# wvu-navLab/corenav-GP

Hardware: AMD Instinct MI355X
Metric: GP-fits/s (higher is better)
Workload: dtype f64; 1 GPU; BASELINE configs[1]: batch of independent fixed-theta GP fits, N=2048 d=6 M=599 kernel=SE-ARD f64; streams=0, pipeline_depth=1, N=2048, d=6, M=599, inputs=resident in HBM, ranks=1

## Files before the change

corenav_gp_amd/csrc/cgp_kernels_fused.hpp:

```cpp
#pragma once
#include "cgp_kernels.hpp"

namespace cgp {

#ifndef CGP_SKIP_DEAD_WAVE
#define CGP_SKIP_DEAD_WAVE 1
#endif
constexpr bool kSkipDeadWave = CGP_SKIP_DEAD_WAVE != 0;

template <typename T>
__device__ __forceinline__ void stage_first_chunk(const T *gR, size_t ldR, const T *gC, size_t ldC, T *smem, int tid) {
  constexpr int CH = KT * LDST;
  if constexpr (sizeof(T) == 8) {
    typedef __attribute__((address_space(3))) void lds_void;
    typedef const __attribute__((address_space(1))) void gbl_void;
    const int lane = tid & 63;
    const int wave = __builtin_amdgcn_readfirstlane(tid >> 6);
#pragma unroll
    for (int i = 0; i < KT / 4; ++i) {
      const int col = wave * (KT / 4) + i;
      __builtin_amdgcn_global_load_lds((gbl_void *)(gR + (size_t)col * ldR + lane * 2), (lds_void *)(smem + col * LDST), 16, 0, 0);
      __builtin_amdgcn_global_load_lds((gbl_void *)(gC + (size_t)col * ldC + lane * 2), (lds_void *)(smem + CH + col * LDST), 16, 0, 0);
    }
  } else {
// ... 529 lines not shown
  for (int ks = 0; ks < KT / 4; ++ks) asm volatile("" : "+v"(f.r[S][ks]));
  if constexpr (ISSUE) {
    cpanel_stage<T>(gC, ldC, c + D, smem + ((S + D) % R) * CH, lane, wave);
    rfrag_load<T, (S + D) % R>(f, gRl, ldR, c + D, lq);
  }
  const T *cur = smem + S * CH + lq * LDST + l15;
  T fa[2][NCB];
#pragma unroll
  for (int cb = 0; cb < NCB; ++cb) fa[0][cb] = cur[cb * DB];
#pragma unroll
  for (int ks = 0; ks < KT / 4; ++ks) {
    if (ks + 1 < KT / 4) {
#pragma unroll
      for (int cb = 0; cb < NCB; ++cb) fa[(ks + 1) & 1][cb] = cur[(ks + 1) * 4 * LDST + cb * DB];
    }
    const typename RowFrag<T, R>::vec2 fb = f.r[S][ks];
    if constexpr (ACC) {
      const T zv = zs[ks * 4 + lq];
      ms[0] = __builtin_fma(fb[0], zv, ms[0]);
      ms[1] = __builtin_fma(fb[1], zv, ms[1]);
      ms[2] = __builtin_fma(fb[0], fb[0], ms[2]);
      ms[3] = __builtin_fma(fb[1], fb[1], ms[3]);
    }
#pragma unroll
    for (int cb = 0; cb < NCB; ++cb) {
      acc[cb][0] = P::mfma(fa[ks & 1][cb], fb[0], acc[cb][0]);
      acc[cb][1] = P::mfma(fa[ks & 1][cb], fb[1], acc[cb][1]);
    }
  }
}

template <typename T, int R = 4>
__device__ __forceinline__ void mfma_rowpanel_loop_rdirect(typename Prec<T>::acc_t (&acc)[NCB][2], RowFrag<T, R> &f, const T *gR,
                                                           size_t ldR, const T *gC, size_t ldC, int nchunk, T *smem, int tid,
                                                           const T *zs, T (&ms)[4]) {
  if (nchunk <= 0) return;
  constexpr int D = deep_dist<R>();
  constexpr int L = cpanel_loads<T>() + KT / 4;
  static_assert((D - 1) * L <= 63 && D < R && 8 % R == 0, "ring / distance / vmcnt");
  const int lane = tid & 63;
  const int wave = __builtin_amdgcn_readfirstlane(tid >> 6);
  const T *gRl = gR + wave * 32 + 2 * (lane & 15);
  int c = 0;
  for (; c + 8 < nchunk; c += R) {
    static_for<0, R>([&](auto jc) {
      constexpr int J = decltype(jc)::value;
      rdirect_step<T, R, J, true, (D - 1) * L>(acc, f, gRl, ldR, gC, ldC, c + J, smem, lane, wave);
    });
  }
  static_for<0, 8>([&](auto jc) {
    constexpr int J = decltype(jc)::value;
    constexpr int behind = (D - 1) < (7 - J) ? (D - 1) : (7 - J);
    rdirect_step<T, R, J % R, (J + D < 8), behind * L, true>(acc, f, gRl, ldR, gC, ldC, c + J, smem, lane, wave, zs + J * KT, ms);
  });
}

constexpr int TRI_PD = 2;
__device__ __forceinline__ constexpr int tri_buf(int i) { return i * KT * LDST; }

template <typename T> constexpr int tri_dma_loads() { return sizeof(T) == 8 ? KT / 4 : KT / 2; }
template <typename T, bool DEEP = sizeof(T) == 8>
__device__ __forceinline__ void stage_chunk_tri(const T *gR, size_t ldR, int chunk, T *buf, int tid) {
  if constexpr (DEEP) {
    typedef __attribute__((address_space(3))) void lds_void;
    typedef const __attribute__((address_space(1))) void gbl_void;
    const int lane = tid & 63;
    const int wave = __builtin_amdgcn_readfirstlane(tid >> 6);
#pragma unroll
    for (int i = 0; i < KT / 4; ++i) {
      const int col = wave * (KT / 4) + i;
      const T *src = gR + (size_t)(chunk * KT + col) * ldR;
      if constexpr (sizeof(T) == 8) {
        __builtin_amdgcn_global_load_lds((gbl_void *)(src + lane * 2), (lds_void *)(buf + col * LDST), 16, 0, 0);
      } else {
        __builtin_amdgcn_global_load_lds((gbl_void *)(src + lane), (lds_void *)(buf + col * LDST), 4, 0, 0);
        __builtin_amdgcn_global_load_lds((gbl_void *)(src + 64 + lane), (lds_void *)(buf + col * LDST + 64), 4, 0, 0);
      }
    }
  } else {
    using vec8 = T __attribute__((ext_vector_type(8)));
    const int sc = tid >> 4, sr = (tid & 15) * 8;
    *reinterpret_cast<vec8 *>(buf + sc * LDST + sr) = *reinterpret_cast<const vec8 *>(gR + sr + (size_t)(chunk * KT + sc) * ldR);
  }
}

template <typename T, int W, bool DEEP>
__device__ __forceinline__ void syrk_tri_wave(typename Prec<T>::acc_t (&acc)[NCB][2], const T *gR, size_t ldR, int nchunk,
                                              T *smem, int tid) {
  using P = Prec<T>;
  constexpr int RB0 = W, RB1 = NCB - 1 - W;
  const int lane = tid & 63;
  const int l15 = lane & 15, lq = lane >> 4;

  auto compute = [&](const T *cur) {
#pragma unroll
    for (int ks = 0; ks < KT / 4; ++ks) {
      const T *ra = cur + (ks * 4 + lq) * LDST + l15;
      T fa[RB1 + 1];
#pragma unroll
      for (int cb = 0; cb <= RB1; ++cb) fa[cb] = ra[cb * DB];
#pragma unroll
      for (int cb = 0; cb <= RB1; ++cb) {
        if (cb <= RB0) acc[cb][0] = P::mfma(fa[cb], fa[RB0], acc[cb][0]);
        acc[cb][1] = P::mfma(fa[cb], fa[RB1], acc[cb][1]);
      }
    }
// ... 96 lines not shown
  const bf8 c01[2] = {__builtin_bit_cast(bf8, a01[RB0]), __builtin_bit_cast(bf8, a01[RB1])};
  static_for<0, RB1 + 1>([&](auto cc) {
    constexpr int CB = decltype(cc)::value;
    const bf8 a = __builtin_bit_cast(bf8, a01[CB]);
    if constexpr (CB <= RB0) acc[CB][0] = __builtin_amdgcn_mfma_f32_16x16x32_bf16(a, c10[0], acc[CB][0], 0, 0, 0);
    acc[CB][1] = __builtin_amdgcn_mfma_f32_16x16x32_bf16(a, c10[1], acc[CB][1], 0, 0, 0);
  });
  static_for<0, RB1 + 1>([&](auto cc) {
    constexpr int CB = decltype(cc)::value;
    const bf8 a = __builtin_bit_cast(bf8, a01[CB]);
    if constexpr (CB <= RB0) acc[CB][0] = __builtin_amdgcn_mfma_f32_16x16x32_bf16(a, c01[0], acc[CB][0], 0, 0, 0);
    acc[CB][1] = __builtin_amdgcn_mfma_f32_16x16x32_bf16(a, c01[1], acc[CB][1], 0, 0, 0);
  });
}
template <int D, int W, int S>
__device__ __forceinline__ void bx6_tri_iter(Prec<float>::acc_t (&acc)[NCB][2], BxTriStage<D> &st, int c, int nchunk, float *smem, const unsigned (&e)[2], bool hi) {
  st.template load<S>(c + D);
  lds_barrier();
  bx6_tri_compute<W, (S & 1) * 6 * BX_PLANE>(acc, e, hi);
  if (c + 1 < nchunk) st.template store<(S + 1) % D>(smem + ((S + 1) & 1) * BXT_FLOATS);
}
template <int D, int W>
__device__ __forceinline__ void bx6_tri_wave(Prec<float>::acc_t (&acc)[NCB][2], BxTriStage<D> &st, int nchunk, float *smem, int tid) {
  const int lane = tid & 63, l15 = lane & 15, lq = lane >> 4;
  const unsigned base = (unsigned)(size_t)smem;
  const unsigned e[2] = {base + 2 * bx_pos(l15, lq & 1), base + 2 * (bx_pos(DB + l15, lq & 1) - DB * BXS)};
  st.template store<0>(smem);
  for (int c0 = 0; c0 < nchunk; c0 += D) {
    bx6_tri_iter<D, W, 0>(acc, st, c0, nchunk, smem, e, lq >> 1);
    bx6_tri_iter<D, W, 1>(acc, st, c0 + 1, nchunk, smem, e, lq >> 1);
    if (D > 2) bx6_tri_iter<D, W, 2 % D>(acc, st, c0 + 2, nchunk, smem, e, lq >> 1);
    if (D > 2) bx6_tri_iter<D, W, 3 % D>(acc, st, c0 + 3, nchunk, smem, e, lq >> 1);
  }
}
template <int D>
__device__ __forceinline__ void bx6_syrk_tri_loop(Prec<float>::acc_t (&acc)[NCB][2], BxTriStage<D> &st, int nchunk, float *smem, int tid) {
  if (nchunk <= 0) return;
  const int wave = __builtin_amdgcn_readfirstlane(tid >> 6);
  switch (wave) {
    case 0: bx6_tri_wave<D, 0>(acc, st, nchunk, smem, tid); break;
    case 1: bx6_tri_wave<D, 1>(acc, st, nchunk, smem, tid); break;
    case 2: bx6_tri_wave<D, 2>(acc, st, nchunk, smem, tid); break;
    default: bx6_tri_wave<D, 3>(acc, st, nchunk, smem, tid); break;
  }
}

__device__ __forceinline__ double exp_gen(double x, const ExpC &e) { return exp_nonpos(x, e); }
__device__ __forceinline__ float exp_gen(float x, const ExpC &) { return __expf(fmaxf(x, -104.f)); }

constexpr int GK = 12;
template <bool DBL> constexpr int bx_z_offset() { return DBL ? 2 * BX_FLOATS : BX_FLOATS + 2 * GK * TS + 3 * TS; }
static_assert(2 * GK * TS + 3 * TS <= BX_FLOATS, "Gram inputs fit the second plane buffer");

template <typename T, bool BROWN, bool FAST, bool TRI = false, int NR = 2, bool DIFF1 = false, int MAT = 0>
__device__ __forceinline__ void gram_apply_tile(const FitArgs &p, typename Prec<T>::acc_t (&acc)[NCB][NR],
                                                const T *__restrict__ xrT, const T *__restrict__ xcT,
                                                const T *__restrict__ xraw, const T *__restrict__ craw,
                                                const T *__restrict__ yc, bool extra, int rowbase, int colbase, T amp,
                                                T amp_b, T diag_add, int lane, int wave, T inv_ell = T(0)) {
  using P = Prec<T>;
  using acc_t = typename P::acc_t;
  const int N = p.N, M = p.M, l15 = lane & 15, lq = lane >> 4;
  ExpC ec;
  ec.load();
  static_assert(NR == 2 || (NR == 1 && !TRI), "row blocks per wave");
  const int rbj[2] = {TRI ? wave : 0, TRI ? NCB - 1 - wave : 0};
  const int rl[2] = {TRI ? rbj[0] * DB + l15 : (NR == 2 ? wave * 32 + 2 * l15 : wave * DB + l15),
                     TRI ? rbj[1] * DB + l15 : wave * 32 + 2 * l15 + 1};
  T fb[NR][GK / 4];
#pragma unroll
  for (int j = 0; j < NR; ++j)
#pragma unroll
    for (int s = 0; s < GK / 4; ++s) fb[j][s] = xrT[(4 * s + lq) * TS + rl[j]];
  static_assert(!DIFF1 || (!BROWN && sizeof(T) == 4), "the difference form is for the fp32 SE kernels");
  static_assert(MAT == 0 || (!BROWN && !DIFF1 && sizeof(T) == 8), "the Matern kernels are fp64 cases of the inner-product form");
  T xrw[2] = {T(0), T(0)};
  if (BROWN || DIFF1) {
    xrw[0] = xraw[rl[0]];
    if (NR == 2) xrw[1] = xraw[rl[1]];
  }
#pragma unroll
  for (int cb = 0; cb < NCB; ++cb) {
    if (TRI && cb > rbj[0] && cb > rbj[1]) continue;
    T fa[GK / 4];
#pragma unroll
    for (int s = 0; s < GK / 4; ++s) fa[s] = xcT[(4 * s + lq) * TS + cb * DB + l15];
#pragma unroll
    for (int j = 0; j < NR; ++j) {
      if (TRI && cb > rbj[j]) continue;
      acc_t e = acc_t{0, 0, 0, 0};
      if constexpr (!DIFF1) {
#pragma unroll
        for (int s = 0; s < GK / 4; ++s) e = P::mfma(fa[s], fb[j][s], e);
      }
      const int grow = rowbase + rl[j];
#pragma unroll
      for (int r = 0; r < 4; ++r) {
        const int cl = cb * DB + P::drow(lane, r);
        const int gcol = colbase + cl;
        T g;
        if constexpr (DIFF1) {
          const T df = (xrw[j] - craw[cl]) * inv_ell;
          g = amp * exp_gen(T(-0.5) * df * df, ec);
        } else if constexpr (MAT != 0) {
          const bool same = !FAST && !extra && grow == gcol;
          double unused;
          g = amp * T(matern_radial<MAT == 2, false>(same ? 0.0 : -2.0 * (double)e[r], unused, [&](double x) { return exp_nonpos(x, ec); }));
        } else if (!BROWN) {
          g = CGP_DBG_ON(p, 128) ? e[r] : exp_gen(e[r], ec);
        } else {
          const T x = xrw[j], xp = craw[cl];
          const bool same = !FAST && !extra && grow == gcol;
          T ee = e[r] > T(0) ? T(0) : e[r];
          if constexpr (sizeof(T) == 4) {
            const T df = (x - xp) * inv_ell;
            ee = T(-0.5) * df * df;
          }
          ee = same ? T(0) : ee;
          const int sx = (x > T(0)) - (x < T(0)), sp = (xp > T(0)) - (xp < T(0));
          const T ax = x < T(0) ? -x : x, ap = xp < T(0) ? -xp : xp;
          const T kb = (sx == sp) ? amp_b * (ax < ap ? ax : ap) : T(0);
          g = amp * exp_gen(ee, ec) * kb;
        }
        if (!FAST) {
          const bool colok = gcol < N;
          if (!extra) {
            const bool dg = grow == gcol;
            g = dg ? g + diag_add : g;
            g = (grow < N && colok) ? g : (dg ? T(1) : T(0));
          } else {
            if (p.xid) g = (grow == gcol) ? T(1) : T(0);
            g = (grow == M) ? yc[cl] : g;
            g = (!colok || grow > M) ? T(0) : g;
          }
        }
        acc[cb][j][r] = -g;
      }
    }
    __builtin_amdgcn_sched_barrier(0);
  }
}

__global__ void k_prep(FitArgs p, int batch, double *prep, int zero_info, int *wready) {
  const int b = blockIdx.x * blockDim.x + threadIdx.x;
  if (b >= batch) return;
  if (zero_info) p.info[b] = 0;
  if (wready) wready[b] = 0;
  const double *th = p.theta + (size_t)b * MAX_THETA;
  double *o = prep + (size_t)b * PREP_N;
  const int kid = p.kernel_id, d = p.d;
  for (int q = 0; q < MAXD; ++q) {
    double s = 0.0;
    if (q < d) s = k_is_ard(kid) ? 1.0 / th[1 + q] : 1.0 / th[1];
    o[q] = s;
  }
  const bool brown = kid == K_RBF_BROWNIAN;
  o[8] = (brown || k_is_matern(kid)) ? 0.0 : log(th[0]);
  o[9] = th[0];
  o[10] = brown ? th[2] : 0.0;
  const int nth = k_ntheta(kid, d);
  o[11] = th[nth - 1] + 1e-8 + (p.jitter ? p.jitter[b] : 0.0);
  for (int q = 12; q < PREP_N; ++q) o[q] = 0.0;
}

template <typename T> struct GramPre {
  T v[MAXD];
  T yv;
};

template <typename T>
__device__ __forceinline__ void gram_prefetch(const FitArgs &p, int b, int k, int rt, int tid, GramPre<T> &g, int row0 = -1) {
  const int d = p.d, N = p.N, M = p.M;
  const bool extra = rt >= p.NT;
  const T *__restrict__ Xb = reinterpret_cast<const T *>(p.X) + (size_t)b * d * N;
  const T *__restrict__ Xsb = reinterpret_cast<const T *>(p.Xs) + (size_t)b * d * M;
  const T *__restrict__ yb = reinterpret_cast<const T *>(p.y) + (size_t)b * N;
  const bool isrow = tid < TS;
  const int r = tid & 127;
  const T *src = Xb;
  int idx, len = N;
  if (isrow) {
    if (!extra) idx = (row0 >= 0 ? row0 : rt * TS) + r;
    else { src = Xsb; idx = (row0 >= 0 ? row0 : (rt - p.NT) * TS) + r; len = M; }
  } else idx = k * TS + r;
  const bool ok = idx < len;
#pragma unroll
  for (int q = 0; q < MAXD; ++q) g.v[q] = (q < d && ok) ? src[(size_t)q * len + idx] : T(0);
  g.yv = (!isrow && ok) ? yb[idx] : T(0);
}

template <typename T, bool TRI = false, int NR = 2, bool MAT = false>
__device__ __forceinline__ void gram_apply(const FitArgs &p, typename Prec<T>::acc_t (&acc)[NCB][NR], T *__restrict__ smem,
                                           int b, int k, int rt, int tid, const GramPre<T> &g, PhaseClock *pc = nullptr,
                                           int slot = 0, int row0 = -1, bool live = true) {
  const double *__restrict__ pr = p.prep + (size_t)b * PREP_N;
  const int kid = p.kernel_id, N = p.N, M = p.M;
  const bool extra = rt >= p.NT;
  const bool brown = kid == K_RBF_BROWNIAN;
  const int lane = tid & 63;
  const int wave = __builtin_amdgcn_readfirstlane(tid >> 6);
  T *xrT = smem;
  T *xcT = smem + GK * TS;
  T *xraw = smem + 2 * GK * TS;
  T *craw = xraw + TS;
  T *yc = craw + TS;
  {
    const bool isrow = tid < TS;
    const int r = tid & 127;
    T *dst = isrow ? xrT : xcT;
    T nrm = 0;
#pragma unroll
    for (int q = 0; q < MAXD; ++q) {
      const T v = g.v[q] * T(pr[q]);
      nrm = __builtin_fma(v, v, nrm);
      dst[q * TS + r] = v;
    }
    dst[MAXD * TS + r] = isrow ? (T(-0.5) * nrm + T(pr[8])) : T(1);
    dst[(MAXD + 1) * TS + r] = isrow ? T(1) : T(-0.5) * nrm;
    dst[(MAXD + 2) * TS + r] = T(0);
    dst[(MAXD + 3) * TS + r] = T(0);
    if (isrow) xraw[r] = g.v[0];
    else {
      craw[r] = g.v[0];
      yc[r] = g.yv;
    }
  }
  __syncthreads();
  if (pc) pc->lap(p, slot);
  const T amp = T(pr[9]), amp_b = T(pr[10]), diag_add = T(pr[11]);
  const int rowbase = row0 >= 0 ? row0 : (extra ? (rt - p.NT) * TS : rt * TS);
  const int colbase = k * TS;
  constexpr int ROWS = NR == 2 ? TS : TS / 2;
  const bool fast = (colbase + TS <= N) && (extra ? (rowbase + ROWS <= M && !p.xid) : (rt != k && rowbase + ROWS <= N));
  if (!live) return;
  if constexpr (sizeof(T) == 4) {
    if (!brown && p.d == 1) {
      if constexpr (TRI) gram_apply_tile<T, false, false, true, NR, true>(p, acc, xrT, xcT, xraw, craw, yc, extra, rowbase, colbase, amp, amp_b, diag_add, lane, wave, T(pr[0]));
      else if (fast) gram_apply_tile<T, false, true, false, NR, true>(p, acc, xrT, xcT, xraw, craw, yc, extra, rowbase, colbase, amp, amp_b, diag_add, lane, wave, T(pr[0]));
      else gram_apply_tile<T, false, false, false, NR, true>(p, acc, xrT, xcT, xraw, craw, yc, extra, rowbase, colbase, amp, amp_b, diag_add, lane, wave, T(pr[0]));
      return;
    }
  }
  static_assert(!MAT || sizeof(T) == 8, "the Matern kernels are fp64 only");
  if constexpr (MAT) {
#define CGP_MATERN_TILE(FAST_, TRI_)                                                                                                  \
  do {                                                                                                                                \
    if (kid == K_MATERN52_ARD)                                                                                                        \
      gram_apply_tile<T, false, FAST_, TRI_, NR, false, 2>(p, acc, xrT, xcT, xraw, craw, yc, extra, rowbase, colbase, amp, amp_b, diag_add, lane, wave); \
    else                                                                                                                              \
      gram_apply_tile<T, false, FAST_, TRI_, NR, false, 1>(p, acc, xrT, xcT, xraw, craw, yc, extra, rowbase, colbase, amp, amp_b, diag_add, lane, wave); \
  } while (0)
    if constexpr (TRI) CGP_MATERN_TILE(false, true);
    else if (fast) CGP_MATERN_TILE(true, false);
    else CGP_MATERN_TILE(false, false);
#undef CGP_MATERN_TILE
    return;
  }
  if constexpr (TRI) {
    if (brown) gram_apply_tile<T, true, false, true>(p, acc, xrT, xcT, xraw, craw, yc, extra, rowbase, colbase, amp, amp_b, diag_add, lane, wave, T(pr[0]));
    else gram_apply_tile<T, false, false, true>(p, acc, xrT, xcT, xraw, craw, yc, extra, rowbase, colbase, amp, amp_b, diag_add, lane, wave);
  } else if (brown) {
    if (fast) gram_apply_tile<T, true, true, false, NR>(p, acc, xrT, xcT, xraw, craw, yc, extra, rowbase, colbase, amp, amp_b, diag_add, lane, wave, T(pr[0]));
    else gram_apply_tile<T, true, false, false, NR>(p, acc, xrT, xcT, xraw, craw, yc, extra, rowbase, colbase, amp, amp_b, diag_add, lane, wave, T(pr[0]));
  } else {
    if (fast) gram_apply_tile<T, false, true, false, NR>(p, acc, xrT, xcT, xraw, craw, yc, extra, rowbase, colbase, amp, amp_b, diag_add, lane, wave);
    else gram_apply_tile<T, false, false, false, NR>(p, acc, xrT, xcT, xraw, craw, yc, extra, rowbase, colbase, amp, amp_b, diag_add, lane, wave);
  }
}

__device__ __forceinline__ constexpr int tri_blk(int i, int j) { return (i * (i + 1) / 2 + j) * DB * DB; }
template <typename T> constexpr int diag_lds_elems() { return 36 * DB * DB + 3 * DB * DB; }

template <typename T>
__device__ __forceinline__ void diag_factor_packed(const FitArgs &p, T *__restrict__ Bk, T *__restrict__ tile, int ld,
                                                   T *__restrict__ Wk, int b, int k, int tid) {
  using P = Prec<T>;
  using acc_t = typename P::acc_t;
  constexpr int NB = TS / DB;
  const int lane = tid & 63;
  const int wave = __builtin_amdgcn_readfirstlane(tid >> 6);
  const int l15 = lane & 15, lq = lane >> 4;
  const int live = p.N - k * TS;
  T *Dv = Bk + 36 * DB * DB;
  T *DvT = Dv + DB * DB;
  int bad = 0;
  for (int jb = 0; jb < NB; ++jb) {
    const int j0 = jb * DB;
    if (wave == 0) {
      T *Djj = Bk + tri_blk(jb, jb);
      T a[DB], w[DB];
      if (j0 < live) {
#pragma unroll
        for (int c = 0; c < DB; ++c) a[c] = Djj[c * DB + l15];
        factor_block16<T>(a, w, bad, k * TS + j0, l15, [&] {
#pragma unroll
          for (int c = 0; c < DB; ++c) a[c] = Djj[c * DB + l15];
        });
      } else {
#pragma unroll
        for (int c = 0; c < DB; ++c) a[c] = w[c] = (c == l15) ? T(1) : T(0);
      }
      if (lane < DB) {
        T *dvt = DvT + (jb & 1) * DB * DB;
#pragma unroll
        for (int i = 0; i < DB; ++i) {
          Dv[l15 * DB + i] = w[i];
          dvt[i * DB + l15] = w[i];
          Wk[wimg_blk(jb, jb) + l15 * DB + i] = -w[i];
        }
#pragma unroll
        for (int c = 0; c < DB; ++c) tile[(size_t)(j0 + c) * ld + j0 + l15] = (l15 >= c) ? a[c] : T(0);
      }
    } else if (jb > 0) {
      const int pj = jb - 1;
      const T *dvt = DvT + (pj & 1) * DB * DB;
      for (int i = jb + wave - 1; i < NB; i += 3) {
        T *blk = Bk + tri_blk(i, pj);
        T fa[4], fb[4];
#pragma unroll
// ... 360 lines not shown
  for (int cb = 0; cb < NCB; ++cb)
#pragma unroll
    for (int r = 0; r < 4; ++r) {
      vec2 v;
      v[0] = acc[cb][0][r];
      v[1] = acc[cb][1][r];
      *reinterpret_cast<vec2 *>(out + (size_t)(cb * DB + P::drow(lane, r)) * ld) = v;
    }
}
template <typename T, bool ADD>
__device__ __forceinline__ void load_tile(typename Prec<T>::acc_t (&acc)[NCB][2], const T *tile, int ld, int tid) {
  using P = Prec<T>;
  using vec2 = T __attribute__((ext_vector_type(2)));
  const int lane = tid & 63, l15 = lane & 15;
  const int wave = __builtin_amdgcn_readfirstlane(tid >> 6);
  const T *src = tile + wave * 32 + 2 * l15;
#pragma unroll
  for (int cb = 0; cb < NCB; ++cb)
#pragma unroll
    for (int r = 0; r < 4; ++r) {
      const vec2 v = *reinterpret_cast<const vec2 *>(src + (size_t)(cb * DB + P::drow(lane, r)) * ld);
      acc[cb][0][r] = ADD ? acc[cb][0][r] + v[0] : v[0];
      acc[cb][1][r] = ADD ? acc[cb][1][r] + v[1] : v[1];
    }
}


template <typename T, bool DEEP, bool MAT = false>
__device__ __forceinline__ void panel_partial(const FitArgs &p, typename Prec<T>::acc_t (&acc)[NCB][2], T *__restrict__ smem, int b,
                                              int k, int tid) {
  constexpr int CH2 = 2 * KT * LDST;
  const int kc = k + 1, rt = k + 2, ld = p.ld, nchunk = k * (TS / KT);
  const T *Lw = reinterpret_cast<const T *>(p.Lw) + (size_t)b * p.lw_stride;
  const T *gR = Lw + (size_t)rt * TS, *gC = Lw + (size_t)kc * TS;
  GramPre<T> gp;
  gram_prefetch<T>(p, b, kc, rt, tid, gp);
  if constexpr (DEEP) {
    constexpr int R = deep_ring<T, true>();
    RowFrag<T, R> rf;
    T *zs = smem + R * KT * LDST;
    if (tid < TS) zs[tid] = T(0);
    T ms[4] = {T(0), T(0), T(0), T(0)};
    rdirect_prologue<T, R>(rf, gR, (size_t)ld, gC, (size_t)ld, nchunk, smem, tid);
    gram_apply<T, false, 2, MAT>(p, acc, smem + (R - 2) * KT * LDST, b, kc, rt, tid, gp);
    mfma_rowpanel_loop_rdirect<T, R>(acc, rf, gR, (size_t)ld, gC, (size_t)ld, nchunk, smem, tid, zs, ms);
  } else {
    if (nchunk > 0) stage_first_chunk<T>(gR, (size_t)ld, gC, (size_t)ld, smem, tid);
    gram_apply<T, false, 2, MAT>(p, acc, smem + CH2, b, kc, rt, tid, gp);
    mfma_rowpanel_loop<T, true>(acc, gR, (size_t)ld, gC, (size_t)ld, nchunk, smem, tid);
  }
  acc_image<T, false, true>(acc, reinterpret_cast<T *>(p.pimg) + ((size_t)b * img_slots(p) + kc % img_slots(p)) * DPART, tid);
}

#ifndef CGP_IMG_EARLY
#define CGP_IMG_EARLY 1
#endif
template <typename T, bool MID> constexpr bool mid_fat() { return MID && sizeof(T) == 4; }
template <typename T, bool DIAGNEXT, bool DEEP, bool MID, bool MAT = false>
__device__ __forceinline__ void panel_tile_body(const FitArgs &p, int k, int b, int rt, int c_first, bool finish_next, bool from_image,
                                                T *smem, int tid) {
  using P = Prec<T>;
  using acc_t = typename P::acc_t;
  acc_t acc[NCB][2];
  T *Lw = reinterpret_cast<T *>(p.Lw) + (size_t)b * p.lw_stride;
  const int ld = p.ld;
  PhaseClock pc;
  pc.start(p, tid);
  const int ps = finish_next ? 336 : 64 + 8 * (k & 31);

  constexpr int CH2 = 2 * KT * LDST;
  const T *gR = Lw + (size_t)rt * TS + (size_t)(c_first * KT) * ld, *gC = Lw + (size_t)k * TS + (size_t)(c_first * KT) * ld;
  if (CGP_DBG_ON(p, 4096)) gR = reinterpret_cast<const T *>(p.Lw) + (size_t)(b & 7) * p.lw_stride + (size_t)p.NT * TS;
  if (CGP_DBG_ON(p, 8192)) gC = reinterpret_cast<const T *>(p.Lw) + (size_t)(b & 7) * p.lw_stride + (size_t)k * TS;
  const int nchunk = k * (TS / KT) - c_first;
  const T *pimg = reinterpret_cast<const T *>(p.pimg) + ((size_t)b * img_slots(p) + k % img_slots(p)) * DPART;
  const bool accm = p.macc != nullptr && rt >= p.NT && k > 0;
  const bool live = !(kSkipDeadWave && !DEEP && sizeof(T) == 4 && rt >= p.NT && !p.xid &&
                      (rt - p.NT) * TS + __builtin_amdgcn_readfirstlane(tid >> 6) * 32 > p.M);
  constexpr int R = DEEP ? deep_ring<T, MID>() : 4;
  constexpr bool BX6 = kF32Bf16x6 && sizeof(T) == 4 && (!DEEP || MID);
  constexpr bool BXDBL = DEEP;
  constexpr int BXD = DEEP ? kBxMidSets : 1;
  constexpr bool PL = kMidPlanes && BX6 && MID;
  constexpr int GRAM_OFF = PL ? 2 * BXP_BUF / 4 : (BX6 ? BX_FLOATS : CH2);
  T *zs = smem + (PL ? BXP_NBUF * BXP_BUF / 4 : (BX6 ? bx_z_offset<BXDBL>() : R * KT * LDST));
  if (tid < TS) zs[tid] = accm ? Lw[(size_t)((k - 1) * TS + tid) * ld + (size_t)p.NT * TS + p.M] : T(0);
  T ms[4] = {T(0), T(0), T(0), T(0)};
  if constexpr (DEEP && !BX6) {
    RowFrag<T, R> rf;
    {
      GramPre<T> gp;
      if (!(MID && from_image)) gram_prefetch<T>(p, b, k, rt, tid, gp);
      rdirect_prologue<T, R>(rf, gR, (size_t)ld, gC, (size_t)ld, nchunk, smem, tid);
      if (MID && from_image) acc_image<T, false, false>(acc, const_cast<T *>(pimg), tid);
      else gram_apply<T, false, 2, MAT>(p, acc, smem + (R - 2) * KT * LDST, b, k, rt, tid, gp, &pc, ps + 6);
    }
    pc.lap(p, ps + 0);
    mfma_rowpanel_loop_rdirect<T, R>(acc, rf, gR, (size_t)ld, gC, (size_t)ld, nchunk, smem, tid, zs, ms);
  } else {
    BxStage<PL ? 1 : BXD> bxs;
    BxPlaneSrc bps;
    {
      GramPre<T> gp;
      if (!(MID && from_image)) gram_prefetch<T>(p, b, k, rt, tid, gp);
      if (nchunk > 0) {
        if constexpr (PL) {
          bps.init(reinterpret_cast<const unsigned short *>(p.Lp) + (size_t)b * p.lp_stride, p.lp_stride / 3, ld, c_first, rt, k, tid);
          const int wv = __builtin_amdgcn_readfirstlane(tid >> 6);
          bps.issue(0, reinterpret_cast<unsigned char *>(smem), 0, wv);
          bps.issue(1, reinterpret_cast<unsigned char *>(smem), BXP_BUF, wv);
        } else if constexpr (BX6) {
          bxs.init(gR, (size_t)ld, gC, (size_t)ld, nchunk, tid);
          bx6_prologue(bxs, nchunk);
        } else stage_first_chunk<T>(gR, (size_t)ld, gC, (size_t)ld, smem, tid);
      }
      if (CGP_DBG_ON(p, 16384)) {
#pragma unroll
        for (int cb = 0; cb < NCB; ++cb)
#pragma unroll
          for (int j = 0; j < 2; ++j)
#pragma unroll
            for (int r = 0; r < 4; ++r) acc[cb][j][r] = gp.v[0];
      } else if (MID && from_image) acc_image<T, false, false>(acc, const_cast<T *>(pimg), tid);
      else gram_apply<T, false, 2, MAT>(p, acc, smem + GRAM_OFF, b, k, rt, tid, gp, &pc, ps + 6, -1, live);
    }
    pc.lap(p, ps + 0);
    if constexpr (PL) bx6p_loop(acc, bps, nchunk, smem, tid, accm ? zs : nullptr, ms, live, gR, (size_t)ld);
    else if constexpr (BX6) bx6_loop<BXD, BXDBL>(acc, bxs, nchunk, smem, tid, accm ? zs : nullptr, ms, live);
    else mfma_rowpanel_loop<T, true>(acc, gR, (size_t)ld, gC, (size_t)ld, nchunk, smem, tid, accm ? zs : nullptr, ms, live);
  }
  pc.lap(p, ps + 1);
  if (accm) {
#pragma unroll
    for (int q = 0; q < 4; ++q) {
      ms[q] += __shfl_xor(ms[q], 16);
      ms[q] += __shfl_xor(ms[q], 32);
    }
    const int lane = tid & 63;
    const int wave = __builtin_amdgcn_readfirstlane(tid >> 6);
    if (lane < 16) {
#pragma unroll
      for (int j = 0; j < 2; ++j) {
        const int m = (rt - p.NT) * TS + wave * 32 + 2 * lane + j;
        if (m < p.M) {
          double *pm = p.macc + (size_t)b * p.M + m, *pv = p.vacc + (size_t)b * p.M + m;
          const double om = k == 1 ? 0.0 : __hip_atomic_load(pm, __ATOMIC_RELAXED, __HIP_MEMORY_SCOPE_AGENT);
          const double ov = k == 1 ? 0.0 : __hip_atomic_load(pv, __ATOMIC_RELAXED, __HIP_MEMORY_SCOPE_AGENT);
          __hip_atomic_store(pm, om + (double)ms[j], __ATOMIC_RELAXED, __HIP_MEMORY_SCOPE_AGENT);
          __hip_atomic_store(pv, ov + (double)ms[2 + j], __ATOMIC_RELAXED, __HIP_MEMORY_SCOPE_AGENT);
        }
      }
    }
  }
  __syncthreads();
  pc.lap(p, ps + 2);
  if (!CGP_DBG_ON(p, 64)) {
    if constexpr (kF32Bf16x6 && kBxTrmm && sizeof(T) == 4) trmm_bx6(p, acc, smem, b, k, tid, &pc, ps + 3, live);
    else trmm_in_registers<T>(p, acc, smem, b, k, tid, &pc, ps + 3, live);
  }
  pc.lap(p, ps + 4);
  if (live && (!CGP_DBG_ON(p, 32768) || acc[0][0][0] == T(12345.678)))
  store_tile<T>(acc, Lw + (size_t)(k * TS) * ld + (size_t)rt * TS, ld, tid);
  if constexpr (PL) {
    if (live) store_tile_planes(acc, reinterpret_cast<unsigned short *>(p.Lp) + (size_t)b * p.lp_stride, p.lp_stride / 3, ld, rt, k, tid);
  }
  pc.lap(p, ps + 5);
  pc.count(p, ps + 7);
  if constexpr (DIAGNEXT) {
    if (finish_next) {
      bool img_ready = false;
      if constexpr (MID && CGP_IMG_EARLY) {
        if (k + 1 >= 3) {
          const T *img = reinterpret_cast<const T *>(p.dpart) + ((size_t)b * img_slots(p) + (k + 1) % img_slots(p)) * DPART;
          acc_image<T, kTriDiag, false>(acc, const_cast<T *>(img), tid);
          img_ready = true;
        }
      }
      diag_next<T, DIAG_FINISH, kTriDiag, DEEP, mid_fat<T, MID>(), MAT>(p, acc, smem, Lw, b, k + 1, tid, &pc, img_ready);
    }
  }
}

#ifndef CGP_KINDA_PRIO
#define CGP_KINDA_PRIO 0
#endif
#ifndef CGP_F32_FULL_OCC
#define CGP_F32_FULL_OCC 4
#endif
constexpr int F32_FULL_OCC = CGP_F32_FULL_OCC;
template <typename T, bool DIAGNEXT = false, bool DEEP = sizeof(T) == 8, bool MID = false, bool MAT = false>
__global__ __launch_bounds__(256, sizeof(T) == 4 ? (DEEP ? ((MID && (CGP_MID_RING > 4 || CGP_F32_BF16X6)) ? 2 : 3) : F32_FULL_OCC) : 2) void k_panel(FitArgs p, int k) {
  using P = Prec<T>;
  using acc_t = typename P::acc_t;
  extern __shared__ __attribute__((aligned(16))) char smem_raw[];
  T *smem = reinterpret_cast<T *>(smem_raw);
  const int tid = threadIdx.x;
// ... 4 lines not shown
  SpanClock sc;
  sc.enter(p, k, tid);
  if constexpr (DIAGNEXT) {
    const int Tg = gridDim.x, B = gridDim.y;
    const int lin = blockIdx.y * Tg + blockIdx.x;
    const int nA = (p.diag_slots & 1) ? B : 0, nB = (p.diag_slots & 2) ? B : 0, nC = (MID && (p.diag_slots & 4)) ? B : 0;
    int ia = -1, io = lin;
    const int stride = p.diag_stride, ablk = nA >> 8, oblk = (Tg * B - nA) >> 8;
    if (nA > 0 && (B & 255) == 0 && stride > 0 && (ablk - 1) * stride < ablk + oblk) {
      const int j = lin >> 8, r = lin & 255;
      const int before = min((j + stride - 1) / stride, ablk);
      if (j % stride == 0 && j / stride < ablk) ia = (j / stride) * 256 + r;
      else io = (j - before) * 256 + r;
    } else if (lin < nA) ia = lin;
    else io = lin - nA;
    if (CGP_DBG_ON(p, 65536) && (ia >= 0 || io < nB)) {
      if (ia < 0) return;
    }
    if (ia >= 0) {
      b = ia;
      rt = k + 1;
      finish_next = !CGP_DBG_ON(p, 65536);
      if constexpr (MID && CGP_KINDA_PRIO > 0) __builtin_amdgcn_s_setprio(CGP_KINDA_PRIO);
      if (MID && (p.diag_slots & 8)) {
        from_image = true;
        c_first = (k - 1) * (TS / KT);
      }
    } else if (io < nB) {
      b = io;
      T *LwB = reinterpret_cast<T *>(p.Lw) + (size_t)b * p.lw_stride;
      diag_next<T, DIAG_PARTIAL, kTriDiag, DEEP, false, MAT>(p, acc, smem, LwB, b, k + 2, tid);
      sc.leave(p, k, tid);
      return;
    } else if (MID && io < nB + nC) {
      panel_partial<T, DEEP, MAT>(p, acc, smem, io - nB, k, tid);
      sc.leave(p, k, tid);
      return;
    } else {
      const int l2 = io - nB - nC, To = Tg - (nA ? 1 : 0) - (nB ? 1 : 0) - (nC ? 1 : 0);
      if ((B & 7) == 0) {
        const int xcd = l2 & 7, slot = l2 >> 3;
        bt = slot % To;
        b = (slot / To) * 8 + xcd;
      } else {
        bt = l2 % To;
        b = l2 / To;
      }
      const int first = k + 1 + (nA ? 1 : 0);
      const int nin = p.NT - first > 0 ? p.NT - first : 0;
      rt = bt < nin ? first + bt : p.NT + (bt - nin);
    }
  } else {
    tile_fit_of_block(bt, b);
    rt = row_tile_of(bt + p.tile_off, k + 1, p.NT, p.rows_from_extra);
  }
  panel_tile_body<T, DIAGNEXT, DEEP, MID, MAT>(p, k, b, rt, c_first, finish_next, from_image, smem, tid);
  sc.leave(p, k, tid);
}

constexpr int HR = TS / 2;
template <typename T, int SLOT>
__device__ __forceinline__ void r16_load(T (&f)[4][KT / 4], const T *gRl, size_t ldR, int chunk, int lq) {
#pragma unroll
  for (int ks = 0; ks < KT / 4; ++ks) {
    const T *src = gRl + (size_t)(chunk * KT + ks * 4 + lq) * ldR;
    if constexpr (sizeof(T) == 8) asm volatile("global_load_dwordx2 %0, %1, off" : "=&v"(f[SLOT][ks]) : "v"(src));
    else asm volatile("global_load_dword %0, %1, off" : "=&v"(f[SLOT][ks]) : "v"(src));
  }
}
template <typename T, int S, bool ISSUE, int WAITN, bool ACC>
__device__ __forceinline__ void r16_step(typename Prec<T>::acc_t (&acc)[NCB][1], T (&f)[4][KT / 4], const T *gRl, size_t ldR, const T *gC,
                                         size_t ldC, int c, T *smem, int lane, int wave, const T *zs, T *ms) {
  using P = Prec<T>;
  constexpr int CH = KT * LDST;
  const int l15 = lane & 15, lq = lane >> 4;
  asm volatile("s_waitcnt vmcnt(%0)\n\ts_barrier" ::"n"(WAITN) : "memory");
#pragma unroll
  for (int ks = 0; ks < KT / 4; ++ks) asm volatile("" : "+v"(f[S][ks]));
  if constexpr (ISSUE) {
    cpanel_stage<T>(gC, ldC, c + 2, smem + ((S + 2) & 3) * CH, lane, wave);
    r16_load<T, (S + 2) & 3>(f, gRl, ldR, c + 2, lq);
  }
  const T *cur = smem + S * CH + lq * LDST + l15;
  T fa[2][NCB];
#pragma unroll
  for (int cb = 0; cb < NCB; ++cb) fa[0][cb] = cur[cb * DB];
#pragma unroll
  for (int ks = 0; ks < KT / 4; ++ks) {
    if (ks + 1 < KT / 4) {
#pragma unroll
      for (int cb = 0; cb < NCB; ++cb) fa[(ks + 1) & 1][cb] = cur[(ks + 1) * 4 * LDST + cb * DB];
    }
    const T fb = f[S][ks];
    if constexpr (ACC) {
      const T zv = zs[ks * 4 + lq];
      ms[0] = __builtin_fma(fb, zv, ms[0]);
      ms[1] = __builtin_fma(fb, fb, ms[1]);
    }
#pragma unroll
    for (int cb = 0; cb < NCB; ++cb) acc[cb][0] = P::mfma(fa[ks & 1][cb], fb, acc[cb][0]);
  }
}

template <typename T, bool MAT = false>
__global__ __launch_bounds__(256, sizeof(T) == 4 ? 4 : 2) void k_rows64(FitArgs p, int k) {
  using P = Prec<T>;
// ... 686 lines not shown
```

Measured before the change: 11250 fits/s.

## Transpose last partial extra tile update to skip dead row blocks

```diff
diff --git a/corenav_gp_amd/csrc/cgp_kernels_fused.hpp b/corenav_gp_amd/csrc/cgp_kernels_fused.hpp
--- a/corenav_gp_amd/csrc/cgp_kernels_fused.hpp
+++ b/corenav_gp_amd/csrc/cgp_kernels_fused.hpp
@@ -605,6 +605,121 @@
     constexpr int J = decltype(jc)::value;
     constexpr int behind = (D - 1) < (7 - J) ? (D - 1) : (7 - J);
     rdirect_step<T, R, J % R, (J + D < 8), behind * L, true>(acc, f, gRl, ldR, gC, ldC, c + J, smem, lane, wave, zs + J * KT, ms);
+  });
+}
+
+#ifndef CGP_LAST_TILE_COLDEAL
+#define CGP_LAST_TILE_COLDEAL 1
+#endif
+constexpr bool kLastTileColDeal = CGP_LAST_TILE_COLDEAL != 0;
+#ifndef CGP_LAST_TILE_ORDER
+#define CGP_LAST_TILE_ORDER 0
+#endif
+__device__ __forceinline__ int coldeal_blocks(const FitArgs &p, int k) {
+  const int nb = 2 * ((p.M + 1 - (p.ET - 1) * TS + 31) / 32);
+  return (kLastTileColDeal && k >= 1 && p.ET > 0 && !p.rows_from_extra && nb <= 6) ? nb : 0;
+}
+
+template <typename T, int NB, int R, int S, bool ISSUE, int WAITN, bool ACC = false>
+__device__ __forceinline__ void coldeal_step(typename Prec<T>::acc_t (&acc)[NB][2], RowFrag<T, R> &f, const T *gCl, size_t ldC,
+                                             const T *gR, size_t ldR, int c, T *smem, int lane, int wave,
+                                             const T *zs = nullptr, T *ms = nullptr) {
+  using P = Prec<T>;
+  constexpr int CH = KT * LDST;
+  constexpr int D = deep_dist<R>();
+  const int l15 = lane & 15, lq = lane >> 4;
+  static_assert(WAITN >= 0 && WAITN <= 63, "vmcnt is a 6-bit counter");
+  asm volatile("s_waitcnt vmcnt(%0)\n\ts_barrier" ::"n"(WAITN) : "memory");
+#pragma unroll
+  for (int ks = 0; ks < KT / 4; ++ks) asm volatile("" : "+v"(f.r[S][ks]));
+  if constexpr (ISSUE) {
+    cpanel_stage<T>(gR, ldR, c + D, smem + ((S + D) % R) * CH, lane, wave);
+    rfrag_load<T, (S + D) % R>(f, gCl, ldC, c + D, lq);
+  }
+  const T *cur = smem + S * CH + lq * LDST + l15;
+  T fa[2][NB];
+#pragma unroll
+  for (int rb = 0; rb < NB; ++rb) fa[0][rb] = cur[rb * DB];
+#pragma unroll
+  for (int ks = 0; ks < KT / 4; ++ks) {
+    if (ks + 1 < KT / 4) {
+#pragma unroll
+      for (int rb = 0; rb < NB; ++rb) fa[(ks + 1) & 1][rb] = cur[(ks + 1) * 4 * LDST + rb * DB];
+    }
+    const typename RowFrag<T, R>::vec2 fb = f.r[S][ks];
+    if constexpr (ACC) {
+      const T zv = zs[ks * 4 + lq];
+      const T v0 = cur[ks * 4 * LDST + wave * DB], v1 = cur[ks * 4 * LDST + (wave + 4) * DB];
+      ms[0] = __builtin_fma(v0, zv, ms[0]);
+      ms[1] = __builtin_fma(v1, zv, ms[1]);
+      ms[2] = __builtin_fma(v0, v0, ms[2]);
+      ms[3] = __builtin_fma(v1, v1, ms[3]);
+    }
+#pragma unroll
+    for (int rb = 0; rb < NB; ++rb) {
+      acc[rb][0] = P::mfma(fa[ks & 1][rb], fb[0], acc[rb][0]);
+      acc[rb][1] = P::mfma(fa[ks & 1][rb], fb[1], acc[rb][1]);
+    }
+  }
+}
+
+template <typename T, int NB, int R = 4>
+__device__ __forceinline__ void mfma_coldeal_loop(typename Prec<T>::acc_t (&acc)[NB][2], RowFrag<T, R> &f, const T *gR, size_t ldR,
+                                                  const T *gC, size_t ldC, int nchunk, T *smem, int tid, const T *zs, T (&ms)[4]) {
+  if (nchunk <= 0) return;
+  constexpr int D = deep_dist<R>();
+  constexpr int L = cpanel_loads<T>() + KT / 4;
+  static_assert((D - 1) * L <= 63 && D < R && 8 % R == 0, "ring / distance / vmcnt");
+  static_assert(NB >= 2 && NB < NCB && NB % 2 == 0, "live row blocks, rounded up to even");
+  const int lane = tid & 63;
+  const int wave = __builtin_amdgcn_readfirstlane(tid >> 6);
+  const T *gCl = gC + wave * 32 + 2 * (lane & 15);
+  int c = 0;
+  for (; c + 8 < nchunk; c += R) {
+    static_for<0, R>([&](auto jc) {
+      constexpr int J = decltype(jc)::value;
+      coldeal_step<T, NB, R, J, true, (D - 1) * L>(acc, f, gCl, ldC, gR, ldR, c + J, smem, lane, wave);
+    });
+  }
+  static_for<0, 8>([&](auto jc) {
+    constexpr int J = decltype(jc)::value;
+    constexpr int behind = (D - 1) < (7 - J) ? (D - 1) : (7 - J);
+    coldeal_step<T, NB, R, J % R, (J + D < 8), behind * L, true>(acc, f, gCl, ldC, gR, ldR, c + J, smem, lane, wave, zs + J * KT, ms);
+  });
+}
+
+template <typename T, int NB>
+__device__ __forceinline__ void coldeal_to_rows(typename Prec<T>::acc_t (&acc)[NCB][2], const typename Prec<T>::acc_t (&cd)[NB][2],
+                                                T *__restrict__ smem, int tid) {
+  using P = Prec<T>;
+  using vec2 = T __attribute__((ext_vector_type(2)));
+  constexpr int LDX = NB * DB + 2;
+  static_assert(64 * LDX <= 4 * KT * LDST, "a pass fits the chunk ring");
+  const int lane = tid & 63, l15 = lane & 15;
+  const int wave = __builtin_amdgcn_readfirstlane(tid >> 6);
+  const bool rows_live = wave * 32 < NB * DB;
+  const T *rowside = smem + wave * 32 + 2 * l15;
+  T *colside = smem + ((wave & 1) * 32 + 2 * l15) * LDX;
+  static_for<0, 2>([&](auto hc) {
+    constexpr int H = decltype(hc)::value;
+    if ((wave >> 1) == H) {
+#pragma unroll
+      for (int rb = 0; rb < NB; ++rb)
+#pragma unroll
+        for (int j = 0; j < 2; ++j)
+#pragma unroll
+          for (int r = 0; r < 4; ++r) colside[j * LDX + rb * DB + P::drow(lane, r)] = cd[rb][j][r];
+    }
+    lds_barrier();
+#pragma unroll
+    for (int cb = 0; cb < 4; ++cb)
+#pragma unroll
+      for (int r = 0; r < 4; ++r) {
+        const vec2 v = rows_live ? *reinterpret_cast<const vec2 *>(rowside + (cb * DB + P::drow(lane, r)) * LDX) : vec2{T(0), T(0)};
+        acc[4 * H + cb][0][r] = v[0];
+        acc[4 * H + cb][1][r] = v[1];
+      }
+    lds_barrier();
   });
 }
 
@@ -807,6 +922,49 @@
 template <bool DBL> constexpr int bx_z_offset() { return DBL ? 2 * BX_FLOATS : BX_FLOATS + 2 * GK * TS + 3 * TS; }
 static_assert(2 * GK * TS + 3 * TS <= BX_FLOATS, "Gram inputs fit the second plane buffer");
 
+template <typename T, bool BROWN, bool FAST, bool DIFF1, int MAT>
+__device__ __forceinline__ T gram_entry(const FitArgs &p, T ev, T xr, int grow, int cl, int gcol, const T *__restrict__ craw,
+                                        const T *__restrict__ yc, bool extra, T amp, T amp_b, T diag_add, T inv_ell, const ExpC &ec) {
+  const int N = p.N, M = p.M;
+  T g;
+  if constexpr (DIFF1) {
+    const T df = (xr - craw[cl]) * inv_ell;
+    g = amp * exp_gen(T(-0.5) * df * df, ec);
+  } else if constexpr (MAT != 0) {
+    const bool same = !FAST && !extra && grow == gcol;
+    double unused;
+    g = amp * T(matern_radial<MAT == 2, false>(same ? 0.0 : -2.0 * (double)ev, unused, [&](double x) { return exp_nonpos(x, ec); }));
+  } else if (!BROWN) {
+    g = CGP_DBG_ON(p, 128) ? ev : exp_gen(ev, ec);
+  } else {
+    const T x = xr, xp = craw[cl];
+    const bool same = !FAST && !extra && grow == gcol;
+    T ee = ev > T(0) ? T(0) : ev;
+    if constexpr (sizeof(T) == 4) {
+      const T df = (x - xp) * inv_ell;
+      ee = T(-0.5) * df * df;
+    }
+    ee = same ? T(0) : ee;
+    const int sx = (x > T(0)) - (x < T(0)), sp = (xp > T(0)) - (xp < T(0));
+    const T ax = x < T(0) ? -x : x, ap = xp < T(0) ? -xp : xp;
+    const T kb = (sx == sp) ? amp_b * (ax < ap ? ax : ap) : T(0);
+    g = amp * exp_gen(ee, ec) * kb;
+  }
+  if (!FAST) {
+    const bool colok = gcol < N;
+    if (!extra) {
+      const bool dg = grow == gcol;
+      g = dg ? g + diag_add : g;
+      g = (grow < N && colok) ? g : (dg ? T(1) : T(0));
+    } else {
+      if (p.xid) g = (grow == gcol) ? T(1) : T(0);
+      g = (grow == M) ? yc[cl] : g;
+      g = (!colok || grow > M) ? T(0) : g;
+    }
+  }
+  return g;
+}
+
 template <typename T, bool BROWN, bool FAST, bool TRI = false, int NR = 2, bool DIFF1 = false, int MAT = 0>
 __device__ __forceinline__ void gram_apply_tile(const FitArgs &p, typename Prec<T>::acc_t (&acc)[NCB][NR],
                                                 const T *__restrict__ xrT, const T *__restrict__ xcT,
@@ -815,7 +973,7 @@
                                                 T amp_b, T diag_add, int lane, int wave, T inv_ell = T(0)) {
   using P = Prec<T>;
   using acc_t = typename P::acc_t;
-  const int N = p.N, M = p.M, l15 = lane & 15, lq = lane >> 4;
+  const int l15 = lane & 15, lq = lane >> 4;
   ExpC ec;
   ec.load();
   static_assert(NR == 2 || (NR == 1 && !TRI), "row blocks per wave");
@@ -852,44 +1010,50 @@
 #pragma unroll
       for (int r = 0; r < 4; ++r) {
         const int cl = cb * DB + P::drow(lane, r);
-        const int gcol = colbase + cl;
-        T g;
-        if constexpr (DIFF1) {
-          const T df = (xrw[j] - craw[cl]) * inv_ell;
-          g = amp * exp_gen(T(-0.5) * df * df, ec);
-        } else if constexpr (MAT != 0) {
-          const bool same = !FAST && !extra && grow == gcol;
-          double unused;
-          g = amp * T(matern_radial<MAT == 2, false>(same ? 0.0 : -2.0 * (double)e[r], unused, [&](double x) { return exp_nonpos(x, ec); }));
-        } else if (!BROWN) {
-          g = CGP_DBG_ON(p, 128) ? e[r] : exp_gen(e[r], ec);
-        } else {
-          const T x = xrw[j], xp = craw[cl];
-          const bool same = !FAST && !extra && grow == gcol;
-          T ee = e[r] > T(0) ? T(0) : e[r];
-          if constexpr (sizeof(T) == 4) {
-            const T df = (x - xp) * inv_ell;
-            ee = T(-0.5) * df * df;
-          }
-          ee = same ? T(0) : ee;
-          const int sx = (x > T(0)) - (x < T(0)), sp = (xp > T(0)) - (xp < T(0));
-          const T ax = x < T(0) ? -x : x, ap = xp < T(0) ? -xp : xp;
-          const T kb = (sx == sp) ? amp_b * (ax < ap ? ax : ap) : T(0);
-          g = amp * exp_gen(ee, ec) * kb;
-        }
-        if (!FAST) {
-          const bool colok = gcol < N;
-          if (!extra) {
-            const bool dg = grow == gcol;
-            g = dg ? g + diag_add : g;
-            g = (grow < N && colok) ? g : (dg ? T(1) : T(0));
-          } else {
-            if (p.xid) g = (grow == gcol) ? T(1) : T(0);
-            g = (grow == M) ? yc[cl] : g;
-            g = (!colok || grow > M) ? T(0) : g;
-          }
-        }
-        acc[cb][j][r] = -g;
+        acc[cb][j][r] = -gram_entry<T, BROWN, FAST, DIFF1, MAT>(p, e[r], xrw[j], grow, cl, colbase + cl, craw, yc, extra, amp, amp_b, diag_add, inv_ell, ec);
+      }
+    }
+    __builtin_amdgcn_sched_barrier(0);
+  }
+}
+
+template <typename T, int NB, bool BROWN, int MAT>
+__device__ __forceinline__ void gram_apply_tile_cols(const FitArgs &p, typename Prec<T>::acc_t (&acc)[NB][2],
+                                                     const T *__restrict__ xrT, const T *__restrict__ xcT,
+                                                     const T *__restrict__ xraw, const T *__restrict__ craw,
+                                                     const T *__restrict__ yc, bool extra, int rowbase, int colbase, T amp,
+                                                     T amp_b, T diag_add, int lane, int wave, T inv_ell) {
+  using P = Prec<T>;
+  using acc_t = typename P::acc_t;
+  static_assert(sizeof(T) == 8, "fp64 only");
+  const int l15 = lane & 15, lq = lane >> 4;
+  ExpC ec;
+  ec.load();
+  const int cl[2] = {wave * 32 + 2 * l15, wave * 32 + 2 * l15 + 1};
+  T fb[2][GK / 4];
+#pragma unroll
+  for (int j = 0; j < 2; ++j)
+#pragma unroll
+    for (int s = 0; s < GK / 4; ++s) fb[j][s] = xcT[(4 * s + lq) * TS + cl[j]];
+#pragma unroll
+  for (int rb = 0; rb < NB; ++rb) {
+    T fa[GK / 4];
+#pragma unroll
+    for (int s = 0; s < GK / 4; ++s) fa[s] = xrT[(4 * s + lq) * TS + rb * DB + l15];
+    T xrw[4] = {T(0), T(0), T(0), T(0)};
+    if (BROWN) {
+#pragma unroll
+      for (int r = 0; r < 4; ++r) xrw[r] = xraw[rb * DB + P::drow(lane, r)];
+    }
+#pragma unroll
+    for (int j = 0; j < 2; ++j) {
+      acc_t e = acc_t{0, 0, 0, 0};
+#pragma unroll
+      for (int s = 0; s < GK / 4; ++s) e = P::mfma(fa[s], fb[j][s], e);
+#pragma unroll
+      for (int r = 0; r < 4; ++r) {
+        const int grow = rowbase + rb * DB + P::drow(lane, r);
+        acc[rb][j][r] = -gram_entry<T, BROWN, false, false, MAT>(p, e[r], xrw[r], grow, cl[j], colbase + cl[j], craw, yc, extra, amp, amp_b, diag_add, inv_ell, ec);
       }
     }
     __builtin_amdgcn_sched_barrier(0);
@@ -944,6 +1108,30 @@
   g.yv = (!isrow && ok) ? yb[idx] : T(0);
 }
 
+template <typename T>
+__device__ __forceinline__ void gram_stage(const double *__restrict__ pr, T *__restrict__ smem, int tid, const GramPre<T> &g) {
+  T *xrT = smem, *xcT = smem + GK * TS, *xraw = smem + 2 * GK * TS, *craw = xraw + TS, *yc = craw + TS;
+  const bool isrow = tid < TS;
+  const int r = tid & 127;
+  T *dst = isrow ? xrT : xcT;
+  T nrm = 0;
+#pragma unroll
+  for (int q = 0; q < MAXD; ++q) {
+    const T v = g.v[q] * T(pr[q]);
+    nrm = __builtin_fma(v, v, nrm);
+    dst[q * TS + r] = v;
+  }
+  dst[MAXD * TS + r] = isrow ? (T(-0.5) * nrm + T(pr[8])) : T(1);
+  dst[(MAXD + 1) * TS + r] = isrow ? T(1) : T(-0.5) * nrm;
+  dst[(MAXD + 2) * TS + r] = T(0);
+  dst[(MAXD + 3) * TS + r] = T(0);
+  if (isrow) xraw[r] = g.v[0];
+  else {
+    craw[r] = g.v[0];
+    yc[r] = g.yv;
+  }
+}
+
 template <typename T, bool TRI = false, int NR = 2, bool MAT = false>
 __device__ __forceinline__ void gram_apply(const FitArgs &p, typename Prec<T>::acc_t (&acc)[NCB][NR], T *__restrict__ smem,
                                            int b, int k, int rt, int tid, const GramPre<T> &g, PhaseClock *pc = nullptr,
@@ -959,27 +1147,7 @@
   T *xraw = smem + 2 * GK * TS;
   T *craw = xraw + TS;
   T *yc = craw + TS;
-  {
-    const bool isrow = tid < TS;
-    const int r = tid & 127;
-    T *dst = isrow ? xrT : xcT;
-    T nrm = 0;
-#pragma unroll
-    for (int q = 0; q < MAXD; ++q) {
-      const T v = g.v[q] * T(pr[q]);
-      nrm = __builtin_fma(v, v, nrm);
-      dst[q * TS + r] = v;
-    }
-    dst[MAXD * TS + r] = isrow ? (T(-0.5) * nrm + T(pr[8])) : T(1);
-    dst[(MAXD + 1) * TS + r] = isrow ? T(1) : T(-0.5) * nrm;
-    dst[(MAXD + 2) * TS + r] = T(0);
-    dst[(MAXD + 3) * TS + r] = T(0);
-    if (isrow) xraw[r] = g.v[0];
-    else {
-      craw[r] = g.v[0];
-      yc[r] = g.yv;
-    }
-  }
+  gram_stage<T>(pr, smem, tid, g);
   __syncthreads();
   if (pc) pc->lap(p, slot);
   const T amp = T(pr[9]), amp_b = T(pr[10]), diag_add = T(pr[11]);
@@ -1020,6 +1188,29 @@
   } else {
     if (fast) gram_apply_tile<T, false, true, false, NR>(p, acc, xrT, xcT, xraw, craw, yc, extra, rowbase, colbase, amp, amp_b, diag_add, lane, wave);
     else gram_apply_tile<T, false, false, false, NR>(p, acc, xrT, xcT, xraw, craw, yc, extra, rowbase, colbase, amp, amp_b, diag_add, lane, wave);
+  }
+}
+
+template <typename T, int NB, bool MAT>
+__device__ __forceinline__ void gram_apply_cols(const FitArgs &p, typename Prec<T>::acc_t (&acc)[NB][2], T *__restrict__ smem, int b,
+                                                int k, int rt, int tid, const GramPre<T> &g, PhaseClock *pc, int slot) {
+  const double *__restrict__ pr = p.prep + (size_t)b * PREP_N;
+  const int kid = p.kernel_id;
+  const int lane = tid & 63;
+  const int wave = __builtin_amdgcn_readfirstlane(tid >> 6);
+  T *xrT = smem, *xcT = smem + GK * TS, *xraw = smem + 2 * GK * TS, *craw = xraw + TS, *yc = craw + TS;
+  gram_stage<T>(pr, smem, tid, g);
+  __syncthreads();
+  if (pc) pc->lap(p, slot);
+  const T amp = T(pr[9]), amp_b = T(pr[10]), diag_add = T(pr[11]);
+  const int rowbase = (rt - p.NT) * TS, colbase = k * TS;
+  if constexpr (MAT) {
+    if (kid == K_MATERN52_ARD) gram_apply_tile_cols<T, NB, false, 2>(p, acc, xrT, xcT, xraw, craw, yc, true, rowbase, colbase, amp, amp_b, diag_add, lane, wave, T(0));
+    else gram_apply_tile_cols<T, NB, false, 1>(p, acc, xrT, xcT, xraw, craw, yc, true, rowbase, colbase, amp, amp_b, diag_add, lane, wave, T(0));
+  } else if (kid == K_RBF_BROWNIAN) {
+    gram_apply_tile_cols<T, NB, true, 0>(p, acc, xrT, xcT, xraw, craw, yc, true, rowbase, colbase, amp, amp_b, diag_add, lane, wave, T(pr[0]));
+  } else {
+    gram_apply_tile_cols<T, NB, false, 0>(p, acc, xrT, xcT, xraw, craw, yc, true, rowbase, colbase, amp, amp_b, diag_add, lane, wave, T(0));
   }
 }
 
@@ -1486,6 +1677,24 @@
   acc_image<T, false, true>(acc, reinterpret_cast<T *>(p.pimg) + ((size_t)b * img_slots(p) + kc % img_slots(p)) * DPART, tid);
 }
 
+template <typename T, int NB, int R, bool MAT>
+__device__ __forceinline__ void coldeal_update(const FitArgs &p, typename Prec<T>::acc_t (&acc)[NCB][2], T *__restrict__ smem, int b,
+                                               int k, int rt, int tid, const T *gR, const T *gC, int ld, int nchunk, const T *zs,
+                                               T (&ms)[4], PhaseClock &pc, int ps) {
+  typename Prec<T>::acc_t cd[NB][2];
+  RowFrag<T, R> rf;
+  {
+    GramPre<T> gp;
+    gram_prefetch<T>(p, b, k, rt, tid, gp);
+    rdirect_prologue<T, R>(rf, gC, (size_t)ld, gR, (size_t)ld, nchunk, smem, tid);
+    gram_apply_cols<T, NB, MAT>(p, cd, smem + (R - 2) * KT * LDST, b, k, rt, tid, gp, &pc, ps + 6);
+  }
+  pc.lap(p, ps + 0);
+  mfma_coldeal_loop<T, NB, R>(cd, rf, gR, (size_t)ld, gC, (size_t)ld, nchunk, smem, tid, zs, ms);
+  lds_barrier();
+  coldeal_to_rows<T, NB>(acc, cd, smem, tid);
+}
+
 #ifndef CGP_IMG_EARLY
 #define CGP_IMG_EARLY 1
 #endif
@@ -1520,17 +1729,29 @@
   T *zs = smem + (PL ? BXP_NBUF * BXP_BUF / 4 : (BX6 ? bx_z_offset<BXDBL>() : R * KT * LDST));
   if (tid < TS) zs[tid] = accm ? Lw[(size_t)((k - 1) * TS + tid) * ld + (size_t)p.NT * TS + p.M] : T(0);
   T ms[4] = {T(0), T(0), T(0), T(0)};
+  int cd_nb = 0;
+  if constexpr (kLastTileColDeal && DEEP && !BX6 && !DIAGNEXT && !MID && sizeof(T) == 8) {
+    const int nb = coldeal_blocks(p, k);
+    if (nb && rt == p.NT + p.ET - 1 && c_first == 0) {
+      cd_nb = nb;
+      if (nb == 6) coldeal_update<T, 6, R, MAT>(p, acc, smem, b, k, rt, tid, gR, gC, ld, nchunk, zs, ms, pc, ps);
+      else if (nb == 4) coldeal_update<T, 4, R, MAT>(p, acc, smem, b, k, rt, tid, gR, gC, ld, nchunk, zs, ms, pc, ps);
+      else coldeal_update<T, 2, R, MAT>(p, acc, smem, b, k, rt, tid, gR, gC, ld, nchunk, zs, ms, pc, ps);
+    }
+  }
   if constexpr (DEEP && !BX6) {
-    RowFrag<T, R> rf;
-    {
-      GramPre<T> gp;
-      if (!(MID && from_image)) gram_prefetch<T>(p, b, k, rt, tid, gp);
-      rdirect_prologue<T, R>(rf, gR, (size_t)ld, gC, (size_t)ld, nchunk, smem, tid);
-      if (MID && from_image) acc_image<T, false, false>(acc, const_cast<T *>(pimg), tid);
-      else gram_apply<T, false, 2, MAT>(p, acc, smem + (R - 2) * KT * LDST, b, k, rt, tid, gp, &pc, ps + 6);
-    }
-    pc.lap(p, ps + 0);
-    mfma_rowpanel_loop_rdirect<T, R>(acc, rf, gR, (size_t)ld, gC, (size_t)ld, nchunk, smem, tid, zs, ms);
+    if (cd_nb == 0) {
+      RowFrag<T, R> rf;
+      {
+        GramPre<T> gp;
+        if (!(MID && from_image)) gram_prefetch<T>(p, b, k, rt, tid, gp);
+        rdirect_prologue<T, R>(rf, gR, (size_t)ld, gC, (size_t)ld, nchunk, smem, tid);
+        if (MID && from_image) acc_image<T, false, false>(acc, const_cast<T *>(pimg), tid);
+        else gram_apply<T, false, 2, MAT>(p, acc, smem + (R - 2) * KT * LDST, b, k, rt, tid, gp, &pc, ps + 6);
+      }
+      pc.lap(p, ps + 0);
+      mfma_rowpanel_loop_rdirect<T, R>(acc, rf, gR, (size_t)ld, gC, (size_t)ld, nchunk, smem, tid, zs, ms);
+    }
   } else {
     BxStage<PL ? 1 : BXD> bxs;
     BxPlaneSrc bps;
@@ -1575,7 +1796,7 @@
     if (lane < 16) {
 #pragma unroll
       for (int j = 0; j < 2; ++j) {
-        const int m = (rt - p.NT) * TS + wave * 32 + 2 * lane + j;
+        const int m = (rt - p.NT) * TS + (cd_nb ? (wave + 4 * j) * DB + lane : wave * 32 + 2 * lane + j);
         if (m < p.M) {
           double *pm = p.macc + (size_t)b * p.M + m, *pv = p.vacc + (size_t)b * p.M + m;
           const double om = k == 1 ? 0.0 : __hip_atomic_load(pm, __ATOMIC_RELAXED, __HIP_MEMORY_SCOPE_AGENT);
@@ -1686,6 +1907,17 @@
     }
   } else {
     tile_fit_of_block(bt, b);
+    if constexpr (CGP_LAST_TILE_ORDER != 0 && kLastTileColDeal && DEEP && !MID && sizeof(T) == 8) {
+      const int Tg = gridDim.x, B = gridDim.y;
+      if (coldeal_blocks(p, k) && (B & 7) == 0 && p.tile_off == 0 && Tg > 1) {
+        const int lin = blockIdx.y * Tg + blockIdx.x;
+        const int xcd = lin & 7, F = B >> 3;
+        const int slot = CGP_LAST_TILE_ORDER == 1 ? (lin >> 3) : ((lin >> 3) + (Tg - 1) * F) % (Tg * F);
+        const bool others = slot < (Tg - 1) * F;
+        bt = others ? slot % (Tg - 1) : Tg - 1;
+        b = (others ? slot / (Tg - 1) : slot - (Tg - 1) * F) * 8 + xcd;
+      }
+    }
     rt = row_tile_of(bt + p.tile_off, k + 1, p.NT, p.rows_from_extra);
   }
   panel_tile_body<T, DIAGNEXT, DEEP, MID, MAT>(p, k, b, rt, c_first, finish_next, from_image, smem, tid);
```

Result: no change. 11280 fits/s, median of 2 (+0.2%).
